# MadDevX/Inverse-Kinematics-PSO-Research

Hardware: AMD Instinct MI355X
Metric: PSO particle-updates/sec + IK solves/sec, 7-DOF 1024-particle swarm (higher is better)
Workload: dtype f32

## Files before the change

### inverse-kinematics-pso-research_amd/csrc/ikpso_device.h

```cpp
#pragma once

#include <hip/hip_runtime.h>
#include <stdint.h>

#include <type_traits>

#include "ikpso_collide.h"
#include "ikpso_params.h"


namespace ikpso {

__host__ __device__ __forceinline__ uint32_t xor3(uint32_t a, uint32_t b, uint32_t c)
{
#if defined(__HIP_DEVICE_COMPILE__)
    return __builtin_amdgcn_bitop3_b32(a, b, c, 0x96);
#else
    return a ^ b ^ c;
#endif
}

__host__ __device__ __forceinline__ uint32_t shl1(uint32_t t)
{
#if defined(__HIP_DEVICE_COMPILE__)
// ... 996 lines not shown
};

template <class Topo, int MODE, int TERMS>
using TipAccFor =
    std::conditional_t<Topo::kDH, TipBackAccDH<Topo, MODE, TERMS>, TipBackAcc<Topo, MODE, TERMS>>;

template <class Topo, int MODE, int TERMS>
__device__ __forceinline__ float fitness(const ChainConsts<Topo::J>& cc, const float* x, const float* rest,
                                         const float* tgt, float* node_pos ,
                                         const float* dhc, const float* soft, const float* pose = nullptr,
                                         const float* axis = nullptr)
{
    static_assert(!(TERMS & (kTermOrient | kTermAim)) ||
                      (Topo::kDH ? kTipBackward<Topo, MODE, TERMS>
                                 : (MODE == IKPSO_ARITH_FAST && (TERMS & kTermRuntime) && !(TERMS & kTermAim))),
                  "the orientation and aim terms: the folded chain's tip-backward builds; the orientation term "
                  "also the Euler topologies' FAST runtime-term builds");
    static_assert((TERMS & (kTermOrient | kTermAim)) != (kTermOrient | kTermAim), "one tip term or the other");
    constexpr int A = Topo::A;
    if constexpr (kTipBackward<Topo, MODE, TERMS>) {
        if (!node_pos) {
            constexpr int J = Topo::J;
            using Acc = TipAccFor<Topo, MODE, TERMS>;
            Acc tb(dhc, soft, pose, axis);
#pragma unroll
            for (int k = 1; k <= J; ++k) tb.angles(k, x + A * (k - 1), rest + A * (k - 1));
#pragma unroll
            for (int k = J; k >= 1; --k) tb.back(cc, k, node_trig<Acc::HW, A>(x + A * (k - 1)));
            return tb.finish(cc, tgt + 3 * (J - 1));
        }
    }
    CandBuf<Topo, TERMS> cb;
    FitnessFor<Topo, MODE, TERMS> acc(cc, dhc, soft, cb.v);
    if constexpr (!Topo::kDH && (TERMS & kTermOrient)) acc.rot = pose;
#pragma unroll
    for (int k = 1; k <= Topo::J; ++k) {
        acc.node(cc, k, x + A * (k - 1), rest + A * (k - 1), tgt + 3 * (k - 1), node_pos);
    }
    return acc.finish(cc);
}

template <class Topo, int MODE, int TERMS>
__device__ __forceinline__ float residual(const ChainConsts<Topo::J>& cc, const float* x, const float* tgt,
                                          const float* dhc = nullptr)
{
    constexpr int J = Topo::J;
    if constexpr (Topo::kDH) {
        FitnessAccDH<Topo, MODE, TERMS> acc(cc, dhc, cc.aux, nullptr);
#pragma unroll
        for (int k = 1; k <= J; ++k) acc.advance(k, x[k - 1]);
        const float dx = tgt[3 * (J - 1) + 0] - acc.px;
        const float dy = tgt[3 * (J - 1) + 1] - acc.py;
        const float dz = tgt[3 * (J - 1) + 2] - acc.pz;
        return sqrtf(dx * dx + dy * dy + dz * dz);
    } else {
        Frame F[J + 1];
        F[0] = origin_frame(cc.m0);
        float r = 0.0f;
#pragma unroll
        for (int k = 1; k <= J; ++k) {
            const int pk = Topo::kGeneric ? cc.parent[k] : Topo::parent(k);
            constexpr int HW = kHwTrig<Topo, MODE, TERMS>;
            if (kOriginFrame<Topo, TERMS> && pk == 0) {
                float sa, ca, sb, cb, sc, cc_;
                sincos_fast<HW>(x[3 * (k - 1)], &sa, &ca);
                sincos_fast<HW>(x[3 * (k - 1) + 1], &sb, &cb);
                sincos_fast<HW>(x[3 * (k - 1) + 2], &sc, &cc_);
                F[k] = root_frame_sc(sa, ca, sb, cb, sc, cc_, link_len<HW>(cc, k));
            } else {
                F[k] = child_frame<MODE, false, HW>(F[pk], x[3 * (k - 1)], x[3 * (k - 1) + 1], x[3 * (k - 1) + 2],
                                                    link_len<HW>(cc, k));
            }
            if (Topo::effector(k) && cc.eff_slot[k] >= 0) {
                const float dx = tgt[3 * (k - 1) + 0] - F[k].px;
                const float dy = tgt[3 * (k - 1) + 1] - F[k].py;
                const float dz = tgt[3 * (k - 1) + 2] - F[k].pz;
                r += sqrtf(dx * dx + dy * dy + dz * dz);
            }
        }
        return r;
    }
}

struct PsoCoef {
    float w, c1, c2;
    float wq, c1q, c2q;
    float wh, c1h, c2h;
};

template <class CC>
__device__ __forceinline__ PsoCoef pso_coef(const CC& cc)
{
    return PsoCoef{cc.w, cc.c1, cc.c2, cc.wq, cc.c1q, cc.c2q, cc.wh, cc.c1h, cc.c2h};
}

template <class Rng, class = void>
struct Prescaled : std::false_type {};
template <class Rng>
struct Prescaled<Rng, std::void_t<decltype(Rng::kPrescaled)>> : std::bool_constant<Rng::kPrescaled> {};

#ifndef IKPSO_INPLACE_V
#define IKPSO_INPLACE_V 1
#endif
__device__ __forceinline__ void fma_into(float& v, float a, float b, float c)
{
#if defined(__HIP_DEVICE_COMPILE__) && IKPSO_INPLACE_V
    asm("v_fma_f32 %0, %1, %2, %3" : "+v"(v) : "v"(a), "v"(b), "v"(c));
#else
    v = __builtin_fmaf(a, b, c);
#endif
}
__device__ __forceinline__ void fma_inplace(float& v, float a, float c)
{
#if defined(__HIP_DEVICE_COMPILE__) && IKPSO_INPLACE_V
    asm("v_fma_f32 %0, %1, %0, %2" : "+v"(v) : "v"(a), "v"(c));
#else
    v = __builtin_fmaf(a, v, c);
#endif
}

template <int MODE, bool INPLACE = false, class Rng>
__device__ __forceinline__ void pso_update(float& x, float& v, float pb, float g, const PsoCoef& k, Rng& rng)
{
    if constexpr (MODE == IKPSO_ARITH_REFERENCE && Prescaled<Rng>::value) {
        const float wr1 = rng.raw();
        const float c1r2 = rng.raw();
        const float c2r3 = rng.raw();
        {
#pragma clang fp contract(off)
            v = wr1 * v + c1r2 * (pb - x) + c2r3 * (g - x);
            x += v;
        }
    } else if constexpr (MODE == IKPSO_ARITH_REFERENCE) {
        const float r1 = rng.uniform();
        const float r2 = rng.uniform();
        const float r3 = rng.uniform();
        {
#pragma clang fp contract(off)
            v = k.w * r1 * v + k.c1 * r2 * (pb - x) + k.c2 * r3 * (g - x);
            x += v;
        }
    } else {
        const float a = rng.scaled(k.wq, k.wh);
        const float b = rng.scaled(k.c1q, k.c1h);
        const float c = rng.scaled(k.c2q, k.c2h);
        if constexpr (INPLACE)
            fma_inplace(v, a, __builtin_fmaf(b, pb - x, c * (g - x)));
        else
            v = __builtin_fmaf(a, v, __builtin_fmaf(b, pb - x, c * (g - x)));
        x += v;
    }
}

template <class Rng>
__device__ __forceinline__ void pso_draw_ahead(float& pa, float& pc, float x, float v, float pb, const PsoCoef& k,
                                               Rng& rng)
{
    const float a = rng.scaled(k.wq, k.wh);
    const float b = rng.scaled(k.c1q, k.c1h);
    pc = rng.scaled(k.c2q, k.c2h);
    pa = __builtin_fmaf(a, v, b * (pb - x));
}
__device__ __forceinline__ void pso_update_ahead(float& x, float& v, float g, float pa, float pc)
{
    fma_into(v, pc, g - x, pa);
    x += v;
}

__device__ __forceinline__ float clamp_ref(float v, float lo, float hi) { return fminf(fmaxf(v, lo), hi); }

template <int MODE, bool BOUNDS_ORDERED = false>
__device__ __forceinline__ float clamp_mode(float v, float lo, float hi)
{
    if constexpr (MODE == IKPSO_ARITH_FAST || BOUNDS_ORDERED) return __builtin_amdgcn_fmed3f(v, lo, hi);
    return clamp_ref(v, lo, hi);
}

__device__ __forceinline__ uint32_t ordered_key(float f)
{
    const uint32_t u = __float_as_uint(f + 0.0f);
    return (u & 0x80000000u) ? ~u : (u | 0x80000000u);
}
__host__ __device__ inline float key_to_float(uint32_t k)
{
    const uint32_t u = (k & 0x80000000u) ? (k & 0x7fffffffu) : ~k;
    float f;
    __builtin_memcpy(&f, &u, 4);
    return f;
}

__device__ __forceinline__ uint32_t wave_min_u32(uint32_t x)
{
    x = min(x, (uint32_t)__builtin_amdgcn_update_dpp((int)0xFFFFFFFF, (int)x, 0xB1, 0xF, 0xF, false));
    x = min(x, (uint32_t)__builtin_amdgcn_update_dpp((int)0xFFFFFFFF, (int)x, 0x4E, 0xF, 0xF, false));
    x = min(x, (uint32_t)__builtin_amdgcn_update_dpp((int)0xFFFFFFFF, (int)x, 0x141, 0xF, 0xF, false));
    x = min(x, (uint32_t)__builtin_amdgcn_update_dpp((int)0xFFFFFFFF, (int)x, 0x140, 0xF, 0xF, false));
    const uint32_t r0 = (uint32_t)__builtin_amdgcn_readlane((int)x, 0);
    const uint32_t r1 = (uint32_t)__builtin_amdgcn_readlane((int)x, 16);
    const uint32_t r2 = (uint32_t)__builtin_amdgcn_readlane((int)x, 32);
    const uint32_t r3 = (uint32_t)__builtin_amdgcn_readlane((int)x, 48);
    return min(min(r0, r1), min(r2, r3));
}

__device__ __forceinline__ uint32_t scalar_min_u32(uint32_t a, uint32_t b)
{
    uint32_t r;
    asm("s_min_u32 %0, %1, %2" : "=s"(r) : "s"(a), "s"(b) : "scc");
    return r;
}
__device__ __forceinline__ uint32_t wave_min_u32_scalar(uint32_t x)
{
    x = min(x, (uint32_t)__builtin_amdgcn_update_dpp((int)0xFFFFFFFF, (int)x, 0xB1, 0xF, 0xF, false));
    x = min(x, (uint32_t)__builtin_amdgcn_update_dpp((int)0xFFFFFFFF, (int)x, 0x4E, 0xF, 0xF, false));
    x = min(x, (uint32_t)__builtin_amdgcn_update_dpp((int)0xFFFFFFFF, (int)x, 0x141, 0xF, 0xF, false));
    x = min(x, (uint32_t)__builtin_amdgcn_update_dpp((int)0xFFFFFFFF, (int)x, 0x140, 0xF, 0xF, false));
    const uint32_t r0 = (uint32_t)__builtin_amdgcn_readlane((int)x, 0);
    const uint32_t r1 = (uint32_t)__builtin_amdgcn_readlane((int)x, 16);
    const uint32_t r2 = (uint32_t)__builtin_amdgcn_readlane((int)x, 32);
    const uint32_t r3 = (uint32_t)__builtin_amdgcn_readlane((int)x, 48);
    return scalar_min_u32(scalar_min_u32(r0, r1), scalar_min_u32(r2, r3));
}

__device__ __forceinline__ int wave_first_lane_eq(uint32_t key, uint32_t wmin)
{
    const uint64_t m = __ballot(key == wmin);
    return (int)__builtin_ctzll(m);
}

__device__ __forceinline__ float uniform_f32(float v)
{
    return __int_as_float(__builtin_amdgcn_readfirstlane(__float_as_int(v)));
}

}
```

### inverse-kinematics-pso-research_amd/csrc/ikpso_resident.h

```cpp
#pragma once

#include <hip/hip_runtime.h>

#include "ikpso_device.h"
#include "ikpso_kernels.h"
#include "ikpso_swarm.h"

namespace ikpso {

constexpr int kTrigAheadMaxD = 30;
#ifndef IKPSO_PRIO_LEVELS_2WAVE
#define IKPSO_PRIO_LEVELS_2WAVE 3
#endif
constexpr int kPrioLevels2Wave = IKPSO_PRIO_LEVELS_2WAVE, kPrioLevels4Wave = 2;

template <int J, int L, bool INV = false>
__device__ __forceinline__ void progress_prio(int k)
{
    static_assert(L == 0 || (L >= 2 && L <= 4), "priority levels: none or 2..4");
    if constexpr (L > 0) {
        switch (INV ? (L * (k - 1)) / J : (L - 1) - (L * (k - 1)) / J) {
        case 3: __builtin_amdgcn_s_setprio(3); break;
        case 2: __builtin_amdgcn_s_setprio(2); break;
        case 1: __builtin_amdgcn_s_setprio(1); break;
        default: __builtin_amdgcn_s_setprio(0); break;
        }
    }
}

template <int BLOCK, bool SPLIT>
struct PbLane {
    static constexpr int kSplit = 65536 / (4 * BLOCK);
    int lo, hi;
    __device__ __forceinline__ static int upper_lane(int tid)
    {
        int h = tid + kSplit * BLOCK;
        asm("" : "+v"(h));
        return h;
    }
    __device__ __forceinline__ int at(int d) const
    {
        return SPLIT && d >= kSplit ? (d - kSplit) * BLOCK + hi : d * BLOCK + lo;
    }
};

template <int MODE, int TERMS, class Topo>
__device__ __forceinline__ float clamp_angle(const ChainConsts<Topo::J>& cc, const SwarmShared<Topo>& sh, int d, float x)
{
    if constexpr (TERMS & kTermUniformBounds)
        return clamp_mode<MODE, true>(x, uniform_lo<TERMS>(cc), uniform_hi<TERMS>(cc));
    else
        return clamp_mode<MODE>(x, sh.lo[d], sh.hi[d]);
}

template <class Topo, int MODE, int TERMS, int BLOCK, bool SPLIT = false, class Rng>
__device__ __forceinline__ void update_node(const ChainConsts<Topo::J>& cc, const SwarmShared<Topo>& sh,
                                            const float* s_pb, const PbLane<BLOCK, SPLIT>& pbl, int k,
                                            float (&x)[Topo::D], float (&v)[Topo::D], const PsoCoef& coef, Rng& rng)
{
    constexpr int A = Topo::A;
#pragma unroll
    for (int ax = 0; ax < A; ++ax) {
        const int d = A * (k - 1) + ax;
        if (kMasked<Topo, TERMS> && !dim_free(cc, d)) continue;
        pso_update<MODE>(x[d], v[d], s_pb[pbl.at(d)], sh.g[d], coef, rng);
        x[d] = clamp_angle<MODE, TERMS>(cc, sh, d, x[d]);
    }
}

template <class Topo, int MODE, int TERMS, int BLOCK, bool SPLIT = false, class Rng>
__device__ __forceinline__ float swarm_step_ahead(const ChainConsts<Topo::J>& cc, SwarmShared<Topo>& sh,
                                                  float* s_pb, const PbLane<BLOCK, SPLIT>& pbl, float (&x)[Topo::D],
                                                  float (&v)[Topo::D], const PsoCoef& coef, Rng& rng,
                                                  const float* pose = nullptr)
{
    constexpr int J = Topo::J, A = Topo::A;
    constexpr int HW = kHwTrig<Topo, MODE, TERMS>;
    CandBuf<Topo, TERMS> cb;
    FitnessFor<Topo, MODE, TERMS> acc(cc, sh.dh, sh.soft, cb.v);
    if constexpr (!Topo::kDH && (TERMS & kTermOrient)) acc.rot = pose;
    progress_prio<J, kPrioLevels4Wave>(1);
    update_node<Topo, MODE, TERMS, BLOCK, SPLIT>(cc, sh, s_pb, pbl, 1, x, v, coef, rng);
    NodeTrig<A> cur = node_trig<HW, A>(x);
#pragma unroll
    for (int k = 1; k <= J; ++k) {
        if (k > 1) progress_prio<J, kPrioLevels4Wave>(k);
        NodeTrig<A> nxt = cur;
        if (k < J) {
            update_node<Topo, MODE, TERMS, BLOCK, SPLIT>(cc, sh, s_pb, pbl, k + 1, x, v, coef, rng);
            nxt = node_trig<HW, A>(x + A * k);
        }
        float rest[A], tgt[3];
#pragma unroll
        for (int ax = 0; ax < A; ++ax) rest[ax] = sh.rest[A * (k - 1) + ax];
#pragma unroll
        for (int c = 0; c < 3; ++c) tgt[c] = Topo::effector(k) ? sh.tgt[3 * (k - 1) + c] : 0.0f;
        acc.node_trig(cc, k, x + A * (k - 1), cur, rest, tgt, nullptr);
        cur = nxt;
        if (!Topo::kDH) __builtin_amdgcn_sched_barrier(0);
    }
    return acc.finish(cc);
}

template <class Topo, int MODE, int TERMS, int BLOCK, int KA = 0, bool INV = false, class Rng>
__device__ __forceinline__ void swarm_step_tip(const ChainConsts<Topo::J>& cc, SwarmShared<Topo>& sh, float* s_pb,
                                               int tid, float (&x)[Topo::D], float (&v)[Topo::D], float& pbf,
                                               const PsoCoef& coef, Rng& rng, const float* pa = nullptr,
                                               const float* pc = nullptr, const float* pose = nullptr,
                                               const float* axis = nullptr)
{
    constexpr int J = Topo::J, A = Topo::A, D = Topo::D;
    constexpr int PL = D > kTrigAheadMaxD ? kPrioLevels2Wave : 0;
    using Acc = TipAccFor<Topo, MODE, TERMS>;
    Acc acc(sh.dh, sh.soft, pose, axis);
    float npb[A], ng[A], nrest[A];
#pragma unroll
    for (int ax = 0; ax < A; ++ax) {
        npb[ax] = s_pb[ax * BLOCK + tid];
        ng[ax] = sh.g[ax];
        nrest[ax] = sh.rest[ax];
    }
#pragma unroll
    for (int k = 1; k <= J; ++k) {
        progress_prio<2 * J, PL, INV>(k);
        float cpb[A], cg[A], crest[A];
#pragma unroll
        for (int ax = 0; ax < A; ++ax) {
            cpb[ax] = npb[ax];
            cg[ax] = ng[ax];
            crest[ax] = nrest[ax];
        }
        if (k < J) {
#pragma unroll
            for (int ax = 0; ax < A; ++ax) {
                const int d = A * k + ax;
                npb[ax] = s_pb[d * BLOCK + tid];
                ng[ax] = sh.g[d];
                nrest[ax] = sh.rest[d];
            }
        }
#pragma unroll
        for (int ax = 0; ax < A; ++ax) {
            const int d = A * (k - 1) + ax;
            if (d < KA)
                pso_update_ahead(x[d], v[d], cg[ax], pa[d], pc[d]);
            else
                pso_update<MODE, true>(x[d], v[d], cpb[ax], cg[ax], coef, rng);
            x[d] = clamp_angle<MODE, TERMS>(cc, sh, d, x[d]);
        }
        acc.angles(k, x + A * (k - 1), crest);
        __builtin_amdgcn_sched_barrier(0);
    }
    NodeTrig<A> cur = node_trig<Acc::HW, A>(x + A * (J - 1));
#pragma unroll
    for (int k = J; k >= 1; --k) {
        progress_prio<2 * J, PL, INV>(2 * J + 1 - k);
        NodeTrig<A> nxt = cur;
        if (k > 1) nxt = node_trig<Acc::HW, A>(x + A * (k - 2));
        acc.back(cc, k, cur);
        cur = nxt;
        if (!Topo::kDH) __builtin_amdgcn_sched_barrier(0);
    }
    float tgt[3];
#pragma unroll
    for (int c = 0; c < 3; ++c) tgt[c] = sh.tgt[3 * (J - 1) + c];
    const float f = acc.finish(cc, tgt);
    if (f < pbf) {
        pbf = f;
#pragma unroll
        for (int d = 0; d < D; ++d) s_pb[d * BLOCK + tid] = x[d];
    }
}

constexpr int kVelLdsSat = 9;
template <class Topo, int MODE, int TERMS>
__host__ __device__ constexpr int kVelLds()
{
    constexpr int D = Topo::D, BLOCK = kResidentMaxThreads<D>();
    if (!(TERMS & kTermColliders) || D > 30) return 0;
    constexpr long spare = 163840L - (long)sizeof(SwarmShared<Topo>) - 256 - (long)D * BLOCK * 4;
    constexpr long k = spare / (BLOCK * 4);
    constexpr int fit = k <= 0 ? 0 : (k >= D ? D : (int)k);
    return kFastSat<Topo, MODE, TERMS> && fit > kVelLdsSat ? kVelLdsSat : fit;
}

#ifndef IKPSO_COLLIDE_RELOAD
#define IKPSO_COLLIDE_RELOAD 1
#endif
template <int J>
__device__ __forceinline__ const ChainConsts<J>& kernarg_cc()
{
    const __attribute__((address_space(4))) char* p =
        (const __attribute__((address_space(4))) char*)__builtin_amdgcn_kernarg_segment_ptr();
    asm volatile("" : "+s"(p));
    return *(const ChainConsts<J>*)(const char*)p;
}

template <class Topo, int MODE, int TERMS, int BLOCK, int KV = 0, bool SPLIT = false, class Rng>
__device__ __forceinline__ void swarm_step(const ChainConsts<Topo::J>& cc, SwarmShared<Topo>& sh, float* s_pb,
                                           int tid, float (&x)[Topo::D], float (&v)[Topo::D], float& pbf,
                                           const PsoCoef& coef, Rng& rng, int tid_upper = 0,
                                           const float* pose = nullptr, const float* axis = nullptr)
{
    constexpr int J = Topo::J, A = Topo::A, D = Topo::D;
    constexpr bool MASK = kMasked<Topo, TERMS>;
    if constexpr (kTipBackward<Topo, MODE, TERMS>) {
        swarm_step_tip<Topo, MODE, TERMS, BLOCK>(cc, sh, s_pb, tid, x, v, pbf, coef, rng, nullptr, nullptr, pose,
                                                 axis);
        return;
    }
    if constexpr (MODE == IKPSO_ARITH_FAST && Topo::D <= kTrigAheadMaxD && !(TERMS & kTermColliders)) {
        const PbLane<BLOCK, SPLIT> pbl{tid, tid_upper};
        const float f = swarm_step_ahead<Topo, MODE, TERMS, BLOCK, SPLIT>(cc, sh, s_pb, pbl, x, v, coef, rng, pose);
        if (f < pbf) {
            pbf = f;
#pragma unroll
            for (int d = 0; d < D; ++d) s_pb[pbl.at(d)] = x[d];
        }
        return;
    }
    CandBuf<Topo, TERMS> cb;
    FitnessFor<Topo, MODE, TERMS> acc(cc, sh.dh, sh.soft, cb.v);
    if constexpr ((TERMS & kTermColliders) && SwarmShared<Topo>::kNear > 0 && !IKPSO_COLLIDE_STATS)
        acc.nearc = sh.near4;
    if constexpr (!Topo::kDH && (TERMS & kTermOrient)) acc.rot = pose;
    float* const s_v = s_pb + D * BLOCK;
    auto load_node = [&](int kk, float (&pb)[A], float (&g)[A], float (&rest)[A], float (&tgt)[3], float (&vv)[A]) {
#pragma unroll
        for (int ax = 0; ax < A; ++ax) {
            const int d = A * (kk - 1) + ax;
            pb[ax] = s_pb[d * BLOCK + tid];
            g[ax] = sh.g[d];
            rest[ax] = sh.rest[d];
            if (d < KV) vv[ax] = s_v[d * BLOCK + tid];
        }
#pragma unroll
        for (int c = 0; c < 3; ++c) tgt[c] = Topo::effector(kk) ? sh.tgt[3 * (kk - 1) + c] : 0.0f;
    };
    float npb[A], ng[A], nrest[A], ntgt[3], nv[A];
    load_node(1, npb, ng, nrest, ntgt, nv);
#pragma unroll
    for (int k = 1; k <= J; ++k) {
        progress_prio<J, (D > kTrigAheadMaxD ? kPrioLevels2Wave : kPrioLevels4Wave)>(k);
        float cpb[A], cg[A], crest[A], ctgt[3], cv[A];
#pragma unroll
        for (int ax = 0; ax < A; ++ax) {
            cpb[ax] = npb[ax];
            cg[ax] = ng[ax];
            crest[ax] = nrest[ax];
            if (A * (k - 1) + ax < KV) cv[ax] = nv[ax];
        }
#pragma unroll
        for (int c = 0; c < 3; ++c) ctgt[c] = ntgt[c];
        if (k < J) load_node(k + 1, npb, ng, nrest, ntgt, nv);
#pragma unroll
        for (int ax = 0; ax < A; ++ax) {
            const int d = A * (k - 1) + ax;
            if (MASK && !dim_free(cc, d)) continue;
            if (d < KV) {
                pso_update<MODE>(x[d], cv[ax], cpb[ax], cg[ax], coef, rng);
                s_v[d * BLOCK + tid] = cv[ax];
            } else {
                pso_update<MODE>(x[d], v[d], cpb[ax], cg[ax], coef, rng);
            }
            x[d] = clamp_angle<MODE, TERMS>(cc, sh, d, x[d]);
        }
        acc.node(cc, k, x + A * (k - 1), crest, ctgt, nullptr);
        if (!Topo::kDH) __builtin_amdgcn_sched_barrier(0);
    }

    const float f = acc.finish_for_update(cc, pbf);
    if (f < pbf) {
        pbf = f;
#pragma unroll
        for (int d = 0; d < D; ++d) s_pb[d * BLOCK + tid] = x[d];
    }
}

template <class Topo, int TERMS, int BLOCK, class Rng>
__device__ __forceinline__ void init_particle(const ChainConsts<Topo::J>& cc, const SwarmShared<Topo>& sh,
                                              float* s_pb, int tid, float (&x)[Topo::D], float (&v)[Topo::D],
                                              Rng& rng)
{
#pragma unroll
    for (int d = 0; d < Topo::D; ++d) {
        x[d] = sh.rest[d];
        if (kMasked<Topo, TERMS> && !dim_free(cc, d))
            v[d] = 0.0f;
        else if constexpr (TERMS & kTermRev)
            v[d] = __builtin_fmaf(rng.uniform(), 0.318309886183790672f, -kInv2Pi);
        else
            v[d] = __builtin_fmaf(rng.uniform(), 2.0f, -1.0f);
        s_pb[d * BLOCK + tid] = x[d];
    }
}

#ifndef IKPSO_UNROLL_ITERATIONS
#define IKPSO_UNROLL_ITERATIONS 1
#endif
template <class Topo, int MODE, int TERMS, bool STOP>
constexpr bool kUnrollIterations = IKPSO_UNROLL_ITERATIONS && !STOP && MODE == IKPSO_ARITH_FAST &&
                                   Topo::D <= kTrigAheadMaxD && !(TERMS & kTermColliders) &&
                                   (TERMS & kTermUnitBounds) && !kTipBackward<Topo, MODE, TERMS>;

template <class Topo, int MODE, int TERMS, bool TUNED, class Rng>
__device__ __forceinline__ void resident_iteration(const ChainConsts<Topo::J>& cc, SwarmShared<Topo>& sh, float* s_pb,
                                                   int tid, int tid_upper, int wave, bool active, const PsoCoef& coef,
                                                   int par, float (&x)[Topo::D], float (&v)[Topo::D], float& pbf,
                                                   Rng& rng, uint32_t& gkey, int& bidx, const float* pose = nullptr,
                                                   const float* axis = nullptr)
{
    constexpr int BLOCK = kResidentMaxThreads<Topo::D>();
    constexpr int KV = kVelLds<Topo, MODE, TERMS>();
    compiler_fence();
    if constexpr ((TERMS & kTermColliders) && IKPSO_COLLIDE_RELOAD) {
        const ChainConsts<Topo::J>& cci = kernarg_cc<Topo::J>();
        swarm_step<Topo, MODE, TERMS, BLOCK, KV>(cci, sh, s_pb, tid, x, v, pbf, pso_coef(cci), rng);
    } else {
        swarm_step<Topo, MODE, TERMS, BLOCK, KV, TUNED>(cc, sh, s_pb, tid, x, v, pbf, coef, rng, tid_upper, pose,
                                                        axis);
    }

    const uint32_t bmin = swarm_argmin<TUNED>(sh, par, active ? ordered_key(pbf) : 0xFFFFFFFFu, &bidx, wave);
    if (bmin < gkey) {
        gkey = bmin;
        if constexpr (TUNED)
            copy_gbest<Topo, BLOCK>(sh, s_pb, bidx, wave);
        else
            copy_gbest<Topo, BLOCK>(sh, s_pb, bidx);
        __syncthreads();
    }
}

template <class Topo, int MODE, int TERMS, bool STOP>
__device__ __forceinline__ void swarm_resident_body(const ChainConsts<Topo::J>& cc, const SwarmIO& io,
                                                    SwarmShared<Topo>& sh, float* const s_pb)
{
    constexpr int D = Topo::D;
    constexpr int BLOCK = kResidentMaxThreads<D>();
    const int64_t b = blockIdx.x;
    const int tid = threadIdx.x;
    const int P = io.P;
    const bool active = tid < P;

    stage_swarm_inputs<Topo, TERMS>(cc, io.targets, io.start_pose, b, sh);

    RngFor<TERMS> rng{0, 0, 0, 0, 0, 0};
    if (active) load_rng(rng, io.rng + b * P + tid);
    __syncthreads();

    float x[D], v[D];
    init_particle<Topo, TERMS, BLOCK>(cc, sh, s_pb, tid, x, v, rng);
    constexpr int KV = kVelLds<Topo, MODE, TERMS>();
    float* const s_v = s_pb + D * BLOCK;
#pragma unroll
    for (int d = 0; d < KV; ++d) s_v[d * BLOCK + tid] = v[d];
    float pbf = fitness<Topo, MODE, TERMS>(cc, x, sh.rest, sh.tgt, nullptr, sh.dh, sh.soft);

    int bidx;
    uint32_t gkey = swarm_argmin(sh, 0, active ? ordered_key(pbf) : 0xFFFFFFFFu, &bidx);
    copy_gbest<Topo, BLOCK>(sh, s_pb, bidx);
    __syncthreads();

    const PsoCoef coef = pso_coef(cc);
    constexpr bool UNROLL = kUnrollIterations<Topo, MODE, TERMS, STOP>;
    const int wave = UNROLL ? wave_id_pinned() : 0;
    const int tid_upper = UNROLL ? PbLane<BLOCK, UNROLL>::upper_lane(tid) : 0;
    int it = 0;
    if constexpr (UNROLL) {
        for (; it + 2 <= io.iterations; it += 2) {
            resident_iteration<Topo, MODE, TERMS, UNROLL>(cc, sh, s_pb, tid, tid_upper, wave, active, coef, 1, x, v,
                                                          pbf, rng, gkey, bidx);
            resident_iteration<Topo, MODE, TERMS, UNROLL>(cc, sh, s_pb, tid, tid_upper, wave, active, coef, 0, x, v,
                                                          pbf, rng, gkey, bidx);
        }
        if (it < io.iterations) {
            resident_iteration<Topo, MODE, TERMS, UNROLL>(cc, sh, s_pb, tid, tid_upper, wave, active, coef, 1, x, v,
                                                          pbf, rng, gkey, bidx);
            ++it;
        }
    } else {
        for (; it < io.iterations && (!STOP || gkey > io.stop_key); ++it)
            resident_iteration<Topo, MODE, TERMS, UNROLL>(cc, sh, s_pb, tid, tid_upper, wave, active, coef,
                                                          (it + 1) & 1, x, v, pbf, rng, gkey, bidx);
    }

    compiler_fence();
    store_angles<Topo, TERMS>(cc, io.out_angles, b, tid, tid < D ? sh.g[tid] : 0.0f);
    if (tid == 0 && io.out_fitness) io.out_fitness[b] = key_to_float(gkey);
    if constexpr (STOP) {
        if (tid == 0 && io.out_iterations) io.out_iterations[b] = it;
    }
    if (io.out_residual && tid < 64) {
        float g[D];
#pragma unroll
        for (int d = 0; d < D; ++d) g[d] = sh.g[d];
        const float r = residual<Topo, MODE, TERMS>(cc, g, sh.tgt, sh.dh);
        if (tid == 0) io.out_residual[b] = r;
    }
    if (active) {
        store_rng(rng, io.rng + b * P + tid);
        if (io.dump_particles) {
            float* base = io.dump_particles + b * (int64_t)3 * D * P;
#pragma unroll
            for (int d = 0; d < D; ++d) {
                base[(int64_t)d * P + tid] = radians<TERMS>(x[d]);
                base[(int64_t)(D + d) * P + tid] = radians<TERMS>(d < KV ? s_v[d * BLOCK + tid] : v[d]);
                base[(int64_t)(2 * D + d) * P + tid] = radians<TERMS>(s_pb[d * BLOCK + tid]);
            }
        }
        if (io.dump_bests) io.dump_bests[b * P + tid] = pbf;
    }
}


template <class Topo, int MODE, int TERMS>
__device__ __forceinline__ void swarm_track_body(const ChainConsts<Topo::J>& cc, const SwarmIO& io,
                                                 SwarmShared<Topo>& sh, float* const s_pb, float* const pose = nullptr)
{
    constexpr int D = Topo::D;
    constexpr int BLOCK = kResidentMaxThreads<D>();
    constexpr int KV = kVelLds<Topo, MODE, TERMS>();
    constexpr float sc = (TERMS & kTermRev) ? kInv2Pi : 1.0f;
    const int64_t b = blockIdx.x;
    const int tid = threadIdx.x;
    const int P = io.P;
    const bool active = tid < P;

    for (int d = tid; d < D; d += blockDim.x) {
        sh.lo[d] = cc.lo[d] * sc;
        sh.hi[d] = cc.hi[d] * sc;
        sh.rest[d] =
            (io.start_pose && dim_free(cc, d) ? io.start_pose[b * cc.dfree + dim_rank(cc, d)] : cc.rest[d]) * sc;
    }
    stage_chain_uniforms<Topo, TERMS>(cc, sh);

    RngFor<TERMS> rng{0, 0, 0, 0, 0, 0};
    if (active) load_rng(rng, io.rng + b * P + tid);

    const PsoCoef coef = pso_coef(cc);
    float* const s_v = s_pb + D * BLOCK;
    const float* const axis = (TERMS & kTermAim) ? io.aim_axis : nullptr;
    for (int32_t t = 0; t < io.frames; ++t) {
        const int64_t cell = (int64_t)t * io.num_swarms + b;
        stage_swarm_targets<Topo, TERMS>(cc, io.targets + cell * cc.num_eff * 3, sh);
        if constexpr (TERMS & kTermOrient) {
            if constexpr (Topo::kDH)
                stage_swarm_orientation<Topo>(cc, io, cell, pose);
            else
                stage_swarm_frames<Topo>(cc, io, cell, pose);
        }
        if constexpr (TERMS & kTermAim) stage_swarm_aim<Topo>(cc, io, cell, pose);
        __syncthreads();

        float x[D], v[D];
        init_particle<Topo, TERMS, BLOCK>(cc, sh, s_pb, tid, x, v, rng);
#pragma unroll
        for (int d = 0; d < KV; ++d) s_v[d * BLOCK + tid] = v[d];
        float pbf = fitness<Topo, MODE, TERMS>(cc, x, sh.rest, sh.tgt, nullptr, sh.dh, sh.soft, pose, axis);
        int bidx;
        uint32_t gkey = swarm_argmin(sh, 0, active ? ordered_key(pbf) : 0xFFFFFFFFu, &bidx);
        copy_gbest<Topo, BLOCK>(sh, s_pb, bidx);
        __syncthreads();

        int it = 0;
        for (; it < io.iterations && gkey > io.stop_key; ++it)
            resident_iteration<Topo, MODE, TERMS, false>(cc, sh, s_pb, tid, 0, 0, active, coef, (it + 1) & 1, x, v, pbf,
                                                         rng, gkey, bidx, pose, axis);

        compiler_fence();
        const float answer = tid < D ? answer_angle<Topo, TERMS>(cc, tid, sh.g[tid]) : 0.0f;
        const bool is_free = tid < D && dim_free(cc, tid);
        if (is_free) io.out_angles[cell * cc.dfree + dim_rank(cc, tid)] = answer;
        if (tid == 0 && io.out_fitness) io.out_fitness[cell] = key_to_float(gkey);
        if (tid == 0 && io.out_iterations) io.out_iterations[cell] = it;
        if (io.out_residual && tid < 64) {
            float g[D];
#pragma unroll
            for (int d = 0; d < D; ++d) g[d] = sh.g[d];
            const float r = residual<Topo, MODE, TERMS>(cc, g, sh.tgt, sh.dh);
            if (tid == 0) io.out_residual[cell] = r;
        }
        __syncthreads();
        if (is_free) sh.rest[tid] = answer * sc;
    }
    if (active) store_rng(rng, io.rng + b * P + tid);
}


#ifndef IKPSO_COLLIDE_UNIFORM
#define IKPSO_COLLIDE_UNIFORM 1
#endif

template <class Topo>
constexpr int kResidentMinWaves = Topo::kDH ? 8 : 1;
constexpr size_t kResidentLdsBytes = 160 * 1024;

template <class Topo, int MODE, int TERMS, bool STOP = false, bool TRACK = false>
__global__ void __launch_bounds__(kResidentMaxThreads<Topo::D>(), kResidentMinWaves<Topo>)
    k_swarm_resident(const ChainConsts<Topo::J> cc, const SwarmIO io)
{
    static_assert(STOP || !TRACK, "the track kernel stops per frame");
    constexpr int NPB = (Topo::D + kVelLds<Topo, MODE, TERMS>()) * kResidentMaxThreads<Topo::D>();
    if constexpr (Topo::kGeneric) {
        __shared__ SwarmShared<Topo> sh;
        __shared__ float s_pb[NPB];
        if constexpr (TERMS & kTermOrient) {
            static_assert(TRACK && (TERMS & kTermRuntime), "the effector rotation term: the runtime-term track kernels");
            __shared__ EffFrames<Topo::J> rot;
            static_assert(sizeof(sh) + sizeof(s_pb) + sizeof(rot) <= kResidentLdsBytes, "the workgroup's LDS");
            swarm_track_body<Topo, MODE, TERMS>(cc, io, sh, s_pb, rot.v);
        } else if constexpr (TRACK)
            swarm_track_body<Topo, MODE, TERMS>(cc, io, sh, s_pb);
        else
            swarm_resident_body<Topo, MODE, TERMS, STOP>(cc, io, sh, s_pb);
    } else if constexpr ((TERMS & kTermOrient) && !Topo::kDH) {
        static_assert(TRACK && (TERMS & kTermRuntime), "the effector rotation term: the runtime-term track kernels");
        __shared__ SwarmLds<Topo, NPB, EffFrames<Topo::J>> lds;
        static_assert(sizeof(lds) <= kResidentLdsBytes, "the workgroup's LDS");
        swarm_track_body<Topo, MODE, TERMS>(cc, io, lds.sh, lds.pb, lds.extra.v);
    } else if constexpr (TERMS & (kTermOrient | kTermAim)) {
        static_assert(TRACK && Topo::kDH, "the orientation and aim terms: the folded chain's track kernels");
        static_assert((TERMS & (kTermOrient | kTermAim)) != (kTermOrient | kTermAim), "one tip term or the other");
        __shared__ SwarmLds<Topo, NPB, PoseTarget> lds;
        swarm_track_body<Topo, MODE, TERMS>(cc, io, lds.sh, lds.pb, lds.extra.v);
    } else {
        __shared__ SwarmLds<Topo, NPB> lds;
        if constexpr (TRACK)
            swarm_track_body<Topo, MODE, TERMS>(cc, io, lds.sh, lds.pb);
        else
            swarm_resident_body<Topo, MODE, TERMS, STOP>(cc, io, lds.sh, lds.pb);
    }
}
// ... 81 lines not shown
```

### inverse-kinematics-pso-research_amd/csrc/ikpso_swarm.h

```cpp
#pragma once

#include <hip/hip_runtime.h>

#include "ikpso_device.h"
#include "ikpso_kernels.h"

namespace ikpso {

template <class Rng>
__device__ __forceinline__ void load_rng(Rng& r, const ikpso_rng_state* p)
{
    const uint32_t* q = reinterpret_cast<const uint32_t*>(p);
    r.d = q[0];
    r.v0 = q[1];
    r.v1 = q[2];
    r.v2 = q[3];
    r.v3 = q[4];
    r.v4 = q[5];
}

template <class Rng>
__device__ __forceinline__ void store_rng(const Rng& r, ikpso_rng_state* p)
{
    uint32_t* q = reinterpret_cast<uint32_t*>(p);
// ... 59 lines not shown
__device__ __forceinline__ void stage_swarm_orientation(const ChainConsts<Topo::J>& cc, const SwarmIO& io,
                                                        int64_t cell, float* pose)
{
    if (threadIdx.x != 0) return;
    const float* r = io.target_rot ? io.target_rot + cell * 9 : nullptr;
#pragma unroll
    for (int i = 0; i < 3; ++i) {
        const float r0 = r ? r[3 * i] : 0.0f, r1 = r ? r[3 * i + 1] : 0.0f, r2 = r ? r[3 * i + 2] : 0.0f;
#pragma unroll
        for (int c = 0; c < 3; ++c)
            pose[3 * i + c] = r0 * io.tip_rot[3 * c] + r1 * io.tip_rot[3 * c + 1] + r2 * io.tip_rot[3 * c + 2];
    }
    pose[9] = cc.eff_w[Topo::J] * io.orient_w;
}

template <class Topo>
__device__ __forceinline__ void stage_swarm_aim(const ChainConsts<Topo::J>& cc, const SwarmIO& io, int64_t cell,
                                                float* pose)
{
    if (threadIdx.x != 0) return;
    const float* d = io.aim_dir ? io.aim_dir + cell * 3 : nullptr;
#pragma unroll
    for (int c = 0; c < 3; ++c) pose[c] = d ? d[c] : 0.0f;
    pose[3] = cc.eff_w[Topo::J] * io.aim_w;
}

template <int J>
struct EffFrames {
    float v[kEffFrame * J];
};

template <class Topo>
__device__ __forceinline__ void stage_swarm_frames(const ChainConsts<Topo::J>& cc, const SwarmIO& io, int64_t cell,
                                                   float* rot)
{
    constexpr int J = Topo::J;
    static_assert(J <= kMaxEffFrames, "a weight slot for every node");
    for (int k = threadIdx.x; k < J; k += blockDim.x) {
        const int s = cc.eff_slot[k + 1];
        float rw = 0.0f;
#pragma unroll
        for (int e = 0; e < kMaxEffFrames; ++e) rw = s == e ? io.eff_rot_w[e] : rw;
        const float w = cc.eff_w[k + 1] * rw;
        const float* r = (w != 0.0f && io.eff_rot) ? io.eff_rot + (cell * cc.num_eff + s) * 9 : nullptr;
#pragma unroll
        for (int i = 0; i < 9; ++i) rot[kEffFrame * k + i] = r ? r[i] : 0.0f;
        rot[kEffFrame * k + 9] = r ? w : 0.0f;
    }
}

template <class Topo, int TERMS = 0>
__device__ __forceinline__ void stage_chain_uniforms(const ChainConsts<Topo::J>& cc, SwarmShared<Topo>& sh)
{
    constexpr int J = Topo::J;
    constexpr float sc = (TERMS & kTermRev) ? kInv2Pi : 1.0f;
    if constexpr (Topo::kDH)
        for (int n = threadIdx.x; n < 12 * J + 4; n += blockDim.x) sh.dh[n] = cc.aux[cc.dh_off + n];
    if (cc.use_penalty)
        for (int n = threadIdx.x; n < 6 * J; n += blockDim.x) sh.soft[n] = cc.aux[4 * J + n] * sc;
    if constexpr ((TERMS & kTermColliders) && SwarmShared<Topo>::kNear > 0)
        for (int n = threadIdx.x; n < kNearUnroll * J; n += blockDim.x) {
            const int k = n / kNearUnroll, i = n % kNearUnroll;
            if (i < cc.num_coll) {
                sh.near4[4 * n + 0] = cc.coll[i].px;
                sh.near4[4 * n + 1] = cc.coll[i].py;
                sh.near4[4 * n + 2] = cc.coll[i].pz;
                sh.near4[4 * n + 3] = cc.coll_lim[k * cc.num_coll + i];
            }
        }
}

template <class Topo, int TERMS = 0>
__device__ __forceinline__ void stage_swarm_inputs(const ChainConsts<Topo::J>& cc, const float* targets,
                                                   const float* start_pose, int64_t b, SwarmShared<Topo>& sh)
{
    constexpr int D = Topo::D;
    constexpr float sc = (TERMS & kTermRev) ? kInv2Pi : 1.0f;
    const float* t = targets ? targets + b * (int64_t)cc.num_eff * 3 : nullptr;
    for (int d = threadIdx.x; d < D; d += blockDim.x) {
        sh.lo[d] = cc.lo[d] * sc;
        sh.hi[d] = cc.hi[d] * sc;
        sh.rest[d] = (start_pose && dim_free(cc, d) ? start_pose[b * cc.dfree + dim_rank(cc, d)] : cc.rest[d]) * sc;
    }
    stage_swarm_targets<Topo, TERMS>(cc, t, sh);
    stage_chain_uniforms<Topo, TERMS>(cc, sh);
}

template <int TERMS>
__device__ __forceinline__ float radians(float a)
{
    if constexpr (TERMS & kTermRev)
        return a * k2Pi;
    else
        return a;
}

template <class Topo, int TERMS>
__device__ __forceinline__ float answer_angle(const ChainConsts<Topo::J>& cc, int d, float g)
{
    if constexpr (TERMS & kTermRev) {
        const bool inside = g >= cc.lo[d] * kInv2Pi && g <= cc.hi[d] * kInv2Pi;
        g *= k2Pi;
        if (inside) g = fminf(fmaxf(g, cc.lo[d]), cc.hi[d]);
    }
    return g;
}

template <class Topo, int TERMS = 0>
__device__ __forceinline__ void store_angles(const ChainConsts<Topo::J>& cc, float* out, int64_t b, int d, float g)
{
    if (d < Topo::D && dim_free(cc, d)) out[b * cc.dfree + dim_rank(cc, d)] = answer_angle<Topo, TERMS>(cc, d, g);
}

__device__ __forceinline__ void compiler_fence() { asm volatile("" ::: "memory"); }

struct Planes {
    __amdgpu_buffer_rsrc_t rsrc;
    uint32_t p4;
    uint32_t voff;
    int D;

    __device__ __forceinline__ Planes(float* swarm_base, int D_, int P, int i)
        : rsrc(__builtin_amdgcn_make_buffer_rsrc(swarm_base, 0, 3 * D_ * P * 4, 0x00020000)),
          p4((uint32_t)P * 4u), voff((uint32_t)i * 4u), D(D_)
    {
    }
    __device__ __forceinline__ float ld(int plane, int d) const
    {
        return __uint_as_float(
            __builtin_amdgcn_raw_buffer_load_b32(rsrc, (int)voff, (int)((uint32_t)(plane * D + d) * p4), 0));
    }
    __device__ __forceinline__ void st(int plane, int d, float v) const
    {
        __builtin_amdgcn_raw_buffer_store_b32(__float_as_uint(v), rsrc, (int)voff,
                                              (int)((uint32_t)(plane * D + d) * p4), 0);
    }
};

__device__ __forceinline__ int wave_id() { return __builtin_amdgcn_readfirstlane(threadIdx.x >> 6); }
__device__ __forceinline__ int wave_id_pinned()
{
    int w = wave_id();
    asm("" : "+s"(w));
    return w;
}

__device__ __forceinline__ int lane_id_here()
{
    int lane;
    asm volatile("v_mbcnt_lo_u32_b32 %0, -1, 0\n\tv_mbcnt_hi_u32_b32 %0, -1, %0" : "=v"(lane));
    return lane;
}

template <bool SCALAR = false, class SH>
__device__ __forceinline__ uint32_t swarm_argmin(SH& sh, int par, uint32_t key, int* out_idx, int wave_pinned = 0)
{
    const int lane = lane_id_here(), wave = SCALAR ? wave_pinned : wave_id();
    const int nwaves = blockDim.x >> 6;
    const uint32_t wmin = SCALAR ? wave_min_u32_scalar(key) : wave_min_u32(key);
    const int first = wave_first_lane_eq(key, wmin);
    if (lane == 0) {
        sh.key[par][wave] = wmin;
        sh.idx[par][wave] = wave * 64 + first;
    }
    __syncthreads();
    const uint32_t k2 = lane < nwaves ? sh.key[par][lane] : 0xFFFFFFFFu;
    const uint32_t bmin = SCALAR ? wave_min_u32_scalar(k2) : wave_min_u32(k2);
    *out_idx = __builtin_amdgcn_readfirstlane(sh.idx[par][wave_first_lane_eq(k2, bmin)]);
    return bmin;
}

template <class Topo, int BLOCK>
__device__ __forceinline__ void copy_gbest(SwarmShared<Topo>& sh, const float* s_pb, int idx, int wave)
{
    constexpr int D = Topo::D;
    static_assert(D <= 64, "one wave copies the global best");
    if (wave == 0) {
        const int lane = lane_id_here();
        if (lane < D) sh.g[lane] = s_pb[lane * BLOCK + idx];
    }
}
template <class Topo, int BLOCK>
__device__ __forceinline__ void copy_gbest(SwarmShared<Topo>& sh, const float* s_pb, int idx)
{
    copy_gbest<Topo, BLOCK>(sh, s_pb, idx, wave_id());
}

inline int term_set(const ChainHost& ch)
{
    return (ch.use_posref ? kTermPosRef : 0) | (ch.use_penalty ? kTermPenalty : 0) |
           (ch.uniform_bounds ? kTermUniformBounds : 0) | (ch.num_coll > 0 || ch.poly_trig ? kTermColliders : 0) |
           (ch.masked ? kTermMask : 0);
}

template <class Topo, class F>
inline bool dh_terms(int terms, hipError_t* err, F&& f)
{
    if constexpr (Topo::kDH) {
        switch (terms) {
        case kTermUniformBounds: *err = f(std::integral_constant<int, kTermUniformBounds>{}); return true;
        case kTermUniformBounds | kTermPenalty:
            *err = f(std::integral_constant<int, kTermUniformBounds | kTermPenalty>{});
            return true;
        case 0: *err = f(std::integral_constant<int, 0>{}); return true;
        case kTermPenalty: *err = f(std::integral_constant<int, kTermPenalty>{}); return true;
        default: break;
        }
    }
    (void)terms;
    (void)err;
    return false;
}

template <class Topo, class F>
inline hipError_t with_runtime_terms(const ChainHost& ch, F&& f)
{
    if constexpr (Topo::kDH) {
        return hipErrorNotSupported;
    } else {
        const bool coll = ch.num_coll > 0 || ch.poly_trig;
        if (coll && (ch.masked || (IKPSO_COLLIDE_HW_TRIG && ch.poly_trig) || (ch.num_coll > 0 && !ch.coll_obb)))
            return f(std::integral_constant<int, kTermRuntime | kTermColliders | kTermMask>{});
        if (coll) return f(std::integral_constant<int, kTermRuntime | kTermColliders>{});
        if (ch.masked) return f(std::integral_constant<int, kTermRuntime | kTermMask>{});
        return f(std::integral_constant<int, kTermRuntime>{});
    }
}

template <class F>
inline bool visit_topology(const ChainHost& ch, F&& f)
{
    switch (ch.topo) {
    case TopoKind::Ref7:
#if IKPSO_WITH_REF7
        f(TopoRef7{});
        return true;
#else
        break;
#endif
    case TopoKind::SerialTip:
        switch (ch.J) {
#if IKPSO_WITH_DH
#define IKPSO_S(n) \
    case n: f(TopoSerialTip<n>{}); return true;
            IKPSO_S(6) IKPSO_S(7) IKPSO_S(8) IKPSO_S(9) IKPSO_S(10) IKPSO_S(11) IKPSO_S(12) IKPSO_S(13) IKPSO_S(14)
#undef IKPSO_S
#endif
#if IKPSO_WITH_SERIAL20
        case 20: f(TopoSerialTip<20>{}); return true;
#endif
        default: break;
        }
        break;
    case TopoKind::Generic:
        break;
    case TopoKind::DH:
        switch (ch.J) {
#if IKPSO_WITH_DH
#define IKPSO_D(n) \
    case n: f(TopoDH<n>{}); return true;
            IKPSO_D(3) IKPSO_D(4) IKPSO_D(5) IKPSO_D(6) IKPSO_D(7) IKPSO_D(8) IKPSO_D(9) IKPSO_D(10) IKPSO_D(11)
                IKPSO_D(12)
#undef IKPSO_D
#endif
        default: break;
        }
        return false;
    }
#if IKPSO_WITH_OTHERS
    switch (ch.J) {
#define IKPSO_G(n) \
    case n: f(TopoGeneric<n>{}); return true;
        IKPSO_G(1) IKPSO_G(2) IKPSO_G(3) IKPSO_G(4) IKPSO_G(5) IKPSO_G(6) IKPSO_G(7) IKPSO_G(8) IKPSO_G(9)
            IKPSO_G(10) IKPSO_G(11) IKPSO_G(12) IKPSO_G(13) IKPSO_G(14) IKPSO_G(15) IKPSO_G(16) IKPSO_G(17)
                IKPSO_G(18) IKPSO_G(19) IKPSO_G(20)
#undef IKPSO_G
    default: break;
    }
#endif
    return false;
}


}
```

Measured before the change: 48.61 billion.

## Overlap next-iteration RNG draws with argmin LDS latency in tuned resident loop

Splits the block-wide argmin into a publish phase (barrier plus LDS loads) and a resolve phase. Between them it draws the RNG coefficients for the next iteration's first node, so those draws hide the LDS latency. The second reduction now uses a single DPP row-min, assuming at most 16 waves, instead of a full wave min, and the prefetched draws feed update_node for node 1. This adds registers for the drawn coefficients and restructures the unrolled iteration loop. It risks occupancy loss, and the RNG draw order may change.

```diff
diff --git a/inverse-kinematics-pso-research_amd/csrc/ikpso_device.h b/inverse-kinematics-pso-research_amd/csrc/ikpso_device.h
--- a/inverse-kinematics-pso-research_amd/csrc/ikpso_device.h
+++ b/inverse-kinematics-pso-research_amd/csrc/ikpso_device.h
@@ -1172,6 +1172,24 @@
     }
 }
 
+struct PsoDrawn {
+    float a, b, c;
+};
+template <class Rng>
+__device__ __forceinline__ PsoDrawn pso_draw(const PsoCoef& k, Rng& rng)
+{
+    PsoDrawn r;
+    r.a = rng.scaled(k.wq, k.wh);
+    r.b = rng.scaled(k.c1q, k.c1h);
+    r.c = rng.scaled(k.c2q, k.c2h);
+    return r;
+}
+__device__ __forceinline__ void pso_update_drawn(float& x, float& v, float pb, float g, const PsoDrawn& r)
+{
+    v = __builtin_fmaf(r.a, v, __builtin_fmaf(r.b, pb - x, r.c * (g - x)));
+    x += v;
+}
+
 template <class Rng>
 __device__ __forceinline__ void pso_draw_ahead(float& pa, float& pc, float x, float v, float pb, const PsoCoef& k,
                                                Rng& rng)
@@ -1228,12 +1246,17 @@
     asm("s_min_u32 %0, %1, %2" : "=s"(r) : "s"(a), "s"(b) : "scc");
     return r;
 }
-__device__ __forceinline__ uint32_t wave_min_u32_scalar(uint32_t x)
+__device__ __forceinline__ uint32_t row_min_u32(uint32_t x)
 {
     x = min(x, (uint32_t)__builtin_amdgcn_update_dpp((int)0xFFFFFFFF, (int)x, 0xB1, 0xF, 0xF, false));
     x = min(x, (uint32_t)__builtin_amdgcn_update_dpp((int)0xFFFFFFFF, (int)x, 0x4E, 0xF, 0xF, false));
     x = min(x, (uint32_t)__builtin_amdgcn_update_dpp((int)0xFFFFFFFF, (int)x, 0x141, 0xF, 0xF, false));
     x = min(x, (uint32_t)__builtin_amdgcn_update_dpp((int)0xFFFFFFFF, (int)x, 0x140, 0xF, 0xF, false));
+    return x;
+}
+__device__ __forceinline__ uint32_t wave_min_u32_scalar(uint32_t x)
+{
+    x = row_min_u32(x);
     const uint32_t r0 = (uint32_t)__builtin_amdgcn_readlane((int)x, 0);
     const uint32_t r1 = (uint32_t)__builtin_amdgcn_readlane((int)x, 16);
     const uint32_t r2 = (uint32_t)__builtin_amdgcn_readlane((int)x, 32);
diff --git a/inverse-kinematics-pso-research_amd/csrc/ikpso_resident.h b/inverse-kinematics-pso-research_amd/csrc/ikpso_resident.h
--- a/inverse-kinematics-pso-research_amd/csrc/ikpso_resident.h
+++ b/inverse-kinematics-pso-research_amd/csrc/ikpso_resident.h
@@ -53,18 +53,36 @@
         return clamp_mode<MODE>(x, sh.lo[d], sh.hi[d]);
 }
 
-template <class Topo, int MODE, int TERMS, int BLOCK, bool SPLIT = false, class Rng>
+template <class Topo, int MODE, int TERMS, int BLOCK, bool SPLIT = false, bool DRAWN = false, class Rng>
 __device__ __forceinline__ void update_node(const ChainConsts<Topo::J>& cc, const SwarmShared<Topo>& sh,
                                             const float* s_pb, const PbLane<BLOCK, SPLIT>& pbl, int k,
-                                            float (&x)[Topo::D], float (&v)[Topo::D], const PsoCoef& coef, Rng& rng)
+                                            float (&x)[Topo::D], float (&v)[Topo::D], const PsoCoef& coef, Rng& rng,
+                                            const float* drawn = nullptr)
 {
     constexpr int A = Topo::A;
 #pragma unroll
     for (int ax = 0; ax < A; ++ax) {
         const int d = A * (k - 1) + ax;
         if (kMasked<Topo, TERMS> && !dim_free(cc, d)) continue;
-        pso_update<MODE>(x[d], v[d], s_pb[pbl.at(d)], sh.g[d], coef, rng);
+        if constexpr (DRAWN)
+            pso_update_drawn(x[d], v[d], s_pb[pbl.at(d)], sh.g[d],
+                             PsoDrawn{drawn[3 * ax], drawn[3 * ax + 1], drawn[3 * ax + 2]});
+        else
+            pso_update<MODE>(x[d], v[d], s_pb[pbl.at(d)], sh.g[d], coef, rng);
         x[d] = clamp_angle<MODE, TERMS>(cc, sh, d, x[d]);
+    }
+}
+
+template <class Topo, class Rng>
+__device__ __forceinline__ void draw_node(float* drawn, const PsoCoef& coef, Rng& rng)
+{
+#pragma unroll
+    for (int ax = 0; ax < Topo::A; ++ax) {
+        PsoDrawn r = pso_draw(coef, rng);
+        asm volatile("" : "+v"(r.a), "+v"(r.b), "+v"(r.c));
+        drawn[3 * ax] = r.a;
+        drawn[3 * ax + 1] = r.b;
+        drawn[3 * ax + 2] = r.c;
     }
 }
 
@@ -72,7 +90,7 @@
 __device__ __forceinline__ float swarm_step_ahead(const ChainConsts<Topo::J>& cc, SwarmShared<Topo>& sh,
                                                   float* s_pb, const PbLane<BLOCK, SPLIT>& pbl, float (&x)[Topo::D],
                                                   float (&v)[Topo::D], const PsoCoef& coef, Rng& rng,
-                                                  const float* pose = nullptr)
+                                                  const float* pose = nullptr, const float* node1 = nullptr)
 {
     constexpr int J = Topo::J, A = Topo::A;
     constexpr int HW = kHwTrig<Topo, MODE, TERMS>;
@@ -80,7 +98,7 @@
     FitnessFor<Topo, MODE, TERMS> acc(cc, sh.dh, sh.soft, cb.v);
     if constexpr (!Topo::kDH && (TERMS & kTermOrient)) acc.rot = pose;
     progress_prio<J, kPrioLevels4Wave>(1);
-    update_node<Topo, MODE, TERMS, BLOCK, SPLIT>(cc, sh, s_pb, pbl, 1, x, v, coef, rng);
+    update_node<Topo, MODE, TERMS, BLOCK, SPLIT, SPLIT>(cc, sh, s_pb, pbl, 1, x, v, coef, rng, node1);
     NodeTrig<A> cur = node_trig<HW, A>(x);
 #pragma unroll
     for (int k = 1; k <= J; ++k) {
@@ -200,7 +218,8 @@
 __device__ __forceinline__ void swarm_step(const ChainConsts<Topo::J>& cc, SwarmShared<Topo>& sh, float* s_pb,
                                            int tid, float (&x)[Topo::D], float (&v)[Topo::D], float& pbf,
                                            const PsoCoef& coef, Rng& rng, int tid_upper = 0,
-                                           const float* pose = nullptr, const float* axis = nullptr)
+                                           const float* pose = nullptr, const float* axis = nullptr,
+                                           const float* node1 = nullptr)
 {
     constexpr int J = Topo::J, A = Topo::A, D = Topo::D;
     constexpr bool MASK = kMasked<Topo, TERMS>;
@@ -211,7 +230,7 @@
     }
     if constexpr (MODE == IKPSO_ARITH_FAST && Topo::D <= kTrigAheadMaxD && !(TERMS & kTermColliders)) {
         const PbLane<BLOCK, SPLIT> pbl{tid, tid_upper};
-        const float f = swarm_step_ahead<Topo, MODE, TERMS, BLOCK, SPLIT>(cc, sh, s_pb, pbl, x, v, coef, rng, pose);
+        const float f = swarm_step_ahead<Topo, MODE, TERMS, BLOCK, SPLIT>(cc, sh, s_pb, pbl, x, v, coef, rng, pose, node1);
         if (f < pbf) {
             pbf = f;
 #pragma unroll
@@ -308,7 +327,8 @@
                                                    int tid, int tid_upper, int wave, bool active, const PsoCoef& coef,
                                                    int par, float (&x)[Topo::D], float (&v)[Topo::D], float& pbf,
                                                    Rng& rng, uint32_t& gkey, int& bidx, const float* pose = nullptr,
-                                                   const float* axis = nullptr)
+                                                   const float* axis = nullptr, float* node1 = nullptr,
+                                                   bool more = false)
 {
     constexpr int BLOCK = kResidentMaxThreads<Topo::D>();
     constexpr int KV = kVelLds<Topo, MODE, TERMS>();
@@ -318,10 +338,25 @@
         swarm_step<Topo, MODE, TERMS, BLOCK, KV>(cci, sh, s_pb, tid, x, v, pbf, pso_coef(cci), rng);
     } else {
         swarm_step<Topo, MODE, TERMS, BLOCK, KV, TUNED>(cc, sh, s_pb, tid, x, v, pbf, coef, rng, tid_upper, pose,
-                                                        axis);
-    }
-
-    const uint32_t bmin = swarm_argmin<TUNED>(sh, par, active ? ordered_key(pbf) : 0xFFFFFFFFu, &bidx, wave);
+                                                        axis, node1);
+    }
+
+    uint32_t bmin;
+    if constexpr (TUNED) {
+        static_assert(!kMasked<Topo, TERMS>, "draw_node: every dimension draws");
+        const ArgminPending pend = swarm_argmin_publish(sh, par, active ? ordered_key(pbf) : 0xFFFFFFFFu, wave);
+        progress_prio<Topo::J, kPrioLevels4Wave>(1);
+        if (more) {
+            draw_node<Topo>(node1, coef, rng);
+        } else {
+#pragma unroll
+            for (int n = 0; n < 3 * Topo::A; ++n) node1[n] = 0.0f;
+        }
+        __builtin_amdgcn_sched_barrier(0);
+        bmin = swarm_argmin_resolve(pend, &bidx);
+    } else {
+        bmin = swarm_argmin(sh, par, active ? ordered_key(pbf) : 0xFFFFFFFFu, &bidx);
+    }
     if (bmin < gkey) {
         gkey = bmin;
         if constexpr (TUNED)
@@ -368,17 +403,18 @@
     const int tid_upper = UNROLL ? PbLane<BLOCK, UNROLL>::upper_lane(tid) : 0;
     int it = 0;
     if constexpr (UNROLL) {
-        for (; it + 2 <= io.iterations; it += 2) {
+        float node1[3 * Topo::A];
+        if (io.iterations > 0) draw_node<Topo>(node1, coef, rng);
+        for (; it + 2 < io.iterations; it += 2) {
             resident_iteration<Topo, MODE, TERMS, UNROLL>(cc, sh, s_pb, tid, tid_upper, wave, active, coef, 1, x, v,
-                                                          pbf, rng, gkey, bidx);
+                                                          pbf, rng, gkey, bidx, nullptr, nullptr, node1, true);
             resident_iteration<Topo, MODE, TERMS, UNROLL>(cc, sh, s_pb, tid, tid_upper, wave, active, coef, 0, x, v,
-                                                          pbf, rng, gkey, bidx);
-        }
-        if (it < io.iterations) {
-            resident_iteration<Topo, MODE, TERMS, UNROLL>(cc, sh, s_pb, tid, tid_upper, wave, active, coef, 1, x, v,
-                                                          pbf, rng, gkey, bidx);
-            ++it;
-        }
+                                                          pbf, rng, gkey, bidx, nullptr, nullptr, node1, true);
+        }
+        for (; it < io.iterations; ++it)
+            resident_iteration<Topo, MODE, TERMS, UNROLL>(cc, sh, s_pb, tid, tid_upper, wave, active, coef,
+                                                          (it + 1) & 1, x, v, pbf, rng, gkey, bidx, nullptr, nullptr,
+                                                          node1, it + 1 < io.iterations);
     } else {
         for (; it < io.iterations && (!STOP || gkey > io.stop_key); ++it)
             resident_iteration<Topo, MODE, TERMS, UNROLL>(cc, sh, s_pb, tid, tid_upper, wave, active, coef,
diff --git a/inverse-kinematics-pso-research_amd/csrc/ikpso_swarm.h b/inverse-kinematics-pso-research_amd/csrc/ikpso_swarm.h
--- a/inverse-kinematics-pso-research_amd/csrc/ikpso_swarm.h
+++ b/inverse-kinematics-pso-research_amd/csrc/ikpso_swarm.h
@@ -235,12 +235,12 @@
     return lane;
 }
 
-template <bool SCALAR = false, class SH>
-__device__ __forceinline__ uint32_t swarm_argmin(SH& sh, int par, uint32_t key, int* out_idx, int wave_pinned = 0)
-{
-    const int lane = lane_id_here(), wave = SCALAR ? wave_pinned : wave_id();
+template <class SH>
+__device__ __forceinline__ uint32_t swarm_argmin(SH& sh, int par, uint32_t key, int* out_idx)
+{
+    const int lane = lane_id_here(), wave = wave_id();
     const int nwaves = blockDim.x >> 6;
-    const uint32_t wmin = SCALAR ? wave_min_u32_scalar(key) : wave_min_u32(key);
+    const uint32_t wmin = wave_min_u32(key);
     const int first = wave_first_lane_eq(key, wmin);
     if (lane == 0) {
         sh.key[par][wave] = wmin;
@@ -248,8 +248,39 @@
     }
     __syncthreads();
     const uint32_t k2 = lane < nwaves ? sh.key[par][lane] : 0xFFFFFFFFu;
-    const uint32_t bmin = SCALAR ? wave_min_u32_scalar(k2) : wave_min_u32(k2);
+    const uint32_t bmin = wave_min_u32(k2);
     *out_idx = __builtin_amdgcn_readfirstlane(sh.idx[par][wave_first_lane_eq(k2, bmin)]);
+    return bmin;
+}
+
+struct ArgminPending {
+    uint32_t key;
+    int32_t idx;
+};
+template <class SH>
+__device__ __forceinline__ ArgminPending swarm_argmin_publish(SH& sh, int par, uint32_t key, int wave)
+{
+    static_assert(sizeof(sh.key[0]) == 64 && sizeof(sh.idx[0]) == 64, "16 waves: their keys fill one DPP row");
+    const int lane = lane_id_here();
+    const int nwaves = blockDim.x >> 6;
+    const uint32_t wmin = wave_min_u32_scalar(key);
+    const int first = wave_first_lane_eq(key, wmin);
+    if (lane == 0) {
+        sh.key[par][wave] = wmin;
+        sh.idx[par][wave] = wave * 64 + first;
+    }
+    __syncthreads();
+    ArgminPending p{0xFFFFFFFFu, 0};
+    if (lane < nwaves) {
+        p.key = sh.key[par][lane];
+        p.idx = sh.idx[par][lane];
+    }
+    return p;
+}
+__device__ __forceinline__ uint32_t swarm_argmin_resolve(const ArgminPending& p, int* out_idx)
+{
+    const uint32_t bmin = (uint32_t)__builtin_amdgcn_readlane((int)row_min_u32(p.key), 0);
+    *out_idx = __builtin_amdgcn_readlane(p.idx, wave_first_lane_eq(p.key, bmin));
     return bmin;
 }
 
```

Result: no change. 49.07 billion (median of 6 runs) (+0.9%).
